# justinruggles/flake

Hardware: AMD Instinct MI355X
Metric: Msamples/s encoded, 16-bit stereo 44.1k blocksize 4096 LPC-8 (higher is better)
Workload: dtype int64/f64; 1 GPU; configs[1]: stereo 16-bit 44.1 kHz, blocksize 4096, LPC max order 8 (level-5 params, order method MAX, partition orders 0-5, stereo estimate), synthetic resonator PCM resident in HBM; frames_per_gpu=4096, batches=one resident batch, outputs=subframe info + packed Rice residual sections, parallelism=frame-sharded x1

## Files before the change

flake_amd/csrc/k3_common.h:

```cpp
#pragma once

#include "device_util.h"

namespace fhip {
namespace {

constexpr int ENC_WWORDS = 2048;

__device__ __forceinline__ int clamp_porder(int porder, int n, int order)
{
    int lim = ilog2_dev((uint32_t)(n ^ (n - 1)));
    porder = min(porder, lim);
    if (order > 0) porder = min(porder, ilog2_dev((uint32_t)(n / order)));
    return porder;
}

constexpr int HIST = 32;

template <int C, int T>
struct SmpImg {
    static constexpr bool V4 = (C % 4 == 0);
    static constexpr int CS = V4 ? 4 : 1;
    static constexpr int COL0 = (16 % C == 0) ? HIST / C : (36 + C - 1) / C;
    static constexpr int ROWS = V4 ? C / 4 : C;
    static constexpr int S = T + COL0 + (V4 ? 1 : 2);
    static constexpr int SIZE = ROWS * S * CS;
    __host__ __device__ static constexpr int at(int col, int r)
    {
        return V4 ? ((r / 4) * S + col) * 4 + (r % 4) : r * S + col;
    }
    __host__ __device__ static constexpr int off(int c)
    {
        return at((c - (((c % C) + C) % C)) / C + COL0, ((c % C) + C) % C);
    }
};

struct FastLds {
    int32_t *smp;
    unsigned long long *sums;
    int32_t *kpar;
    double *coefd;
    unsigned long long *wtot;
    uint32_t *lvl_bits, *lvl_meth;
    int32_t *coef;
    int32_t *misc;
    uint32_t *trial;
    uint32_t *bits;
};

__host__ __device__ inline int fast_window_words(int n, bool wide = false)
{
    int w = 256;
    if (wide) { while (w < 2 * ENC_WWORDS && w < n) w <<= 1; return w; }
    while (w < ENC_WWORDS && 2 * w < n) w <<= 1;
    return w;
}
__host__ __device__ inline bool fast_wide_window(int mode, int bps) { return mode == 2 && bps > 16; }

__host__ __device__ inline size_t fast_lds_layout(int n, size_t img_doubles, size_t off[11], bool wide = false)
{
    size_t o = 0;
    off[0] = o; o += 8 * 512;
    off[1] = o; o += 8 * 48;
    off[2] = o; o += 8 * 16;
    off[3] = o; o += 4 * img_doubles;
    off[4] = o; o += 4 * 512;
    off[5] = o; o += 4 * 12;
    off[6] = o; o += 4 * 12;
    off[7] = o; o += 4 * 32;
    off[8] = o; o += 4 * 16;
    off[9] = o; o += 4 * 32;
    o = (o + 15) & ~(size_t)15;
    off[10] = o; o += 4 * fast_window_words(n, wide);
    return o;
}

constexpr int clog2(int v) { return v <= 1 ? 0 : 1 + clog2(v >> 1); }
constexpr int clog2_up(int v) { return clog2(v) + ((v & (v - 1)) ? 1 : 0); }

template <int C, int T>
struct FastCtx {
    FastLds l;
    int n, i0, tid, lane, wv;
    int obits, precision, pmin_req, pmax_req;
};

template <int C, int T, int OBMAX = 8>
__device__ __forceinline__ void fir_lpc(const FastCtx<C, T> &e, int32_t (&r)[C], int order, int shift)
{
    using Img = SmpImg<C, T>;
    const FastLds &l = e.l;
    const double inv = __builtin_ldexp(1.0, -shift);
    constexpr int OB = (C % 8 == 0 && OBMAX >= 8) ? 8 : (C % 4 == 0) ? 4 : (C % 3 == 0) ? 3 : (C % 5 == 0) ? 5 : (C % 7 == 0) ? 7 : 1;
    constexpr int TB = (16 % C == 0) ? 16 : C * ((8 + C - 1) / C);
    const int32_t *mine = l.smp + e.tid * Img::CS;
#pragma unroll
    for (int ob = 0; ob < C; ob += OB) {
        __builtin_amdgcn_sched_barrier(0);
        double acc[OB];
#pragma unroll
        for (int o = 0; o < OB; o++) acc[o] = 0.0;
#pragma unroll 1
        for (int tb = 0; tb < order; tb += TB) {
            const int32_t *base = mine - (tb / C) * Img::CS;
#pragma unroll
            for (int sb = 0; sb < TB; sb += 8) {
                constexpr int dummy = 0; (void)dummy;
                if (order > tb + sb) {
                    const int NT_ = (TB - sb < 8) ? TB - sb : 8;
                    double W[OB + 7];
                    constexpr int WTOP = Img::V4 ? 7 : -1;
                    if constexpr (Img::V4) {
                        static_assert(!Img::V4 || OB % 4 == 0, "aligned windows");
#pragma unroll
                        for (int m4 = 0; m4 < OB + 7; m4 += 4) {
                            const int4 v = *reinterpret_cast<const int4 *>(base + Img::off(ob - sb - 8 + m4));
                            W[m4] = (double)v.x;
                            if (m4 + 1 < OB + 7) W[m4 + 1] = (double)v.y;
                            if (m4 + 2 < OB + 7) W[m4 + 2] = (double)v.z;
                            if (m4 + 3 < OB + 7) W[m4 + 3] = (double)v.w;
                        }
                    } else {
#pragma unroll
                        for (int m = 0; m < OB + 7; m++)
                            if (m < OB + NT_ - 1) W[m] = (double)base[Img::off(ob - sb - NT_ + m)];
                    }
#ifdef FHIP_FIR_TRIM64
                    const int left = order - (tb + sb);
#else
                    constexpr int left = 8;
#endif
#pragma unroll
                    for (int jj = 0; jj < 8; jj++) {
                        if (jj < NT_ && jj < left) {
                            const double cd = l.coefd[tb + sb + jj];
#pragma unroll
                            for (int o = 0; o < OB; o++)
                                acc[o] = __builtin_fma(cd, W[o + (WTOP >= 0 ? WTOP : NT_ - 1) - jj], acc[o]);
                        }
                    }
                }
            }
        }
#pragma unroll
        for (int o = 0; o < OB; o++) {
            const double z = __builtin_fma(acc[o], inv, 6755399441055744.0);
            const uint32_t qlo = (uint32_t)__double2loint(z);
            uint32_t x;
            if constexpr (Img::V4) {
                const int4 v = *reinterpret_cast<const int4 *>(mine + Img::off(ob + (o & ~3)));
                x = (uint32_t)((o & 3) == 0 ? v.x : (o & 3) == 1 ? v.y : (o & 3) == 2 ? v.z : v.w);
            } else {
                x = (uint32_t)mine[Img::off(ob + o)];
            }
            r[ob + o] = (int32_t)(x - qlo);
        }
    }
    if (e.i0 < order) {
#pragma unroll
        for (int o = 0; o < C; o++)
            if (e.i0 + o < order) r[o] = mine[Img::off(o)];
    }
}

template <int C, int T>
__device__ __forceinline__ void fir_lpc_o8(const FastCtx<C, T> &e, int32_t (&r)[C], int order, int shift,
                                           const double *__restrict__ cd)
{
    using Img = SmpImg<C, T>;
    const double inv = __builtin_ldexp(1.0, -shift);
    constexpr int OB = (C % 8 == 0) ? 8 : (C % 4 == 0) ? 4 : (C % 3 == 0) ? 3 : (C % 5 == 0) ? 5 : (C % 7 == 0) ? 7 : 1;
    const int32_t *mine = e.l.smp + e.tid * Img::CS;
    double cf[8];
#pragma unroll
    for (int jj = 0; jj < 8; jj++) cf[jj] = cd[jj];
#pragma unroll
    for (int ob = 0; ob < C; ob += OB) {
        __builtin_amdgcn_sched_barrier(0);
        double acc[OB];
#pragma unroll
        for (int o = 0; o < OB; o++) acc[o] = 0.0;
        double W[OB + 7];
        if constexpr (Img::V4) {
#pragma unroll
            for (int m4 = 0; m4 < OB + 7; m4 += 4) {
                const int4 v = *reinterpret_cast<const int4 *>(mine + Img::off(ob - 8 + m4));
                W[m4] = (double)v.x;
                if (m4 + 1 < OB + 7) W[m4 + 1] = (double)v.y;
                if (m4 + 2 < OB + 7) W[m4 + 2] = (double)v.z;
                if (m4 + 3 < OB + 7) W[m4 + 3] = (double)v.w;
            }
        } else {
#pragma unroll
            for (int m = 0; m < OB + 7; m++) W[m] = (double)mine[Img::off(ob - 8 + m)];
        }
#pragma unroll
        for (int jj = 0; jj < 8; jj++)
#pragma unroll
            for (int o = 0; o < OB; o++)
                acc[o] = __builtin_fma(cf[jj], W[o + 7 - jj], acc[o]);
#pragma unroll
        for (int o = 0; o < OB; o++) {
            const double z = __builtin_fma(acc[o], inv, 6755399441055744.0);
            const uint32_t qlo = (uint32_t)__double2loint(z);
            uint32_t x;
            if constexpr (Img::V4) {
                const int4 v = *reinterpret_cast<const int4 *>(mine + Img::off(ob + (o & ~3)));
                x = (uint32_t)((o & 3) == 0 ? v.x : (o & 3) == 1 ? v.y : (o & 3) == 2 ? v.z : v.w);
            } else {
                x = (uint32_t)mine[Img::off(ob + o)];
            }
            r[ob + o] = (int32_t)(x - qlo);
        }
    }
    if (e.i0 < order) {
#pragma unroll
        for (int o = 0; o < C; o++)
            if (e.i0 + o < order) r[o] = mine[Img::off(o)];
    }
}

template <int C, int T, int TAPS>
__device__ __forceinline__ void fir_lpc_o16(const FastCtx<C, T> &e, int32_t (&r)[C], int order, int shift,
                                            const double *__restrict__ cd)
{
    using Img = SmpImg<C, T>;
// ... 102 lines not shown
```

flake_amd/csrc/k3_encode.hip:

```cpp
#include "device_util.h"
#include "k3_common.h"

#ifdef FHIP_STAMPS
FHIP_DEFINE_STAMP_READER(fhip_debug_read_stamps_k3)
extern "C" int fhip_debug_read_stamps_k1(long long *out);
extern "C" __attribute__((visibility("default"))) int fhip_debug_read_stamps(long long *out)
{
    long long k1[64];
    int rc = fhip_debug_read_stamps_k3(out);
    if (rc == 0) rc = fhip_debug_read_stamps_k1(k1);
    for (int i = 40; i < 64 && rc == 0; i++) out[i] = k1[i];
    return rc;
}
#endif

namespace fhip {
namespace {

struct EncLds {
    int32_t *smp;
    unsigned long long *sums;
    int32_t *kpar;
    uint32_t *lvl_bits;
    uint32_t *lvl_meth;
// ... 1210 lines not shown
            if (ST >= 1) v += row_shl_u64<1>(v);
            if (ST >= 2) v += row_shl_u64<2>(v);
            if (ST >= 3) v += row_shl_u64<4>(v);
            if (ST >= 4) v += row_shl_u64<8>(v);
            if (ST >= 5) v += __shfl_down(v, 16, WAVE);
            if (writer) s5[k * 32 + (tid >> ST)] = v;
        }
    }
    __syncthreads();
    const int pmax_all = clamp_porder(e.pmax_req, n, min_order);
    if (pmax_all <= 3) {
        const int row = lane >> 4, ll = lane & 15;
        for (int slot0 = e.wv * 4; min_order + slot0 <= max_order; slot0 += NW * 4) {
            const int k = min_order + slot0 + row;
            const bool valid = k <= max_order;
            const int kc = min(k, max_order);
            unsigned long long *heap = heaps + (kc - min_order) * 64;
            unsigned long long v = 0;
            if (valid && ll < 8) v = s5[kc * 32 + 4 * ll] + s5[kc * 32 + 4 * ll + 1] + s5[kc * 32 + 4 * ll + 2] + s5[kc * 32 + 4 * ll + 3];
            const bool leaf = valid && ll < 8;
            if (leaf) heap[7 + ll] = v;
            v += row_shl_u64<1>(v); if (leaf && (ll & 1) == 0) heap[3 + (ll >> 1)] = v;
            v += row_shl_u64<2>(v); if (leaf && (ll & 3) == 0) heap[1 + (ll >> 2)] = v;
            v += row_shl_u64<4>(v); if (leaf && ll == 0) heap[0] = v;
            __builtin_amdgcn_fence(__ATOMIC_RELEASE, "wavefront");
            __builtin_amdgcn_wave_barrier();
            const int L = ilog2_dev((uint32_t)n);
            const int lq = (kc == 0) ? 31 : (kc == 1) ? L : (kc == 2) ? L - 1 : (kc == 3) ? ((n >= (3 << (L - 1))) ? L - 1 : L - 2) : L - 2;
            const int lim = min(ilog2_dev((uint32_t)(n ^ (n - 1))), lq);
            const int pmin = min(e.pmin_req, lim), pmax = min(e.pmax_req, lim);
            const int p = ilog2_dev((uint32_t)(ll + 1));
            uint32_t b = 0;
            int kk = 0;
            const unsigned long long hs = heap[min(ll, 14)];
            const unsigned long long total = heap[0];
            if (valid && ll < 15 && p >= pmin && p <= pmax) {
                const int jn = ll + 1 - (1 << p);
                const int cnt = (n >> p) - (jn == 0 ? kc : 0);
                if (total < 0xFFE00000ull && cnt > 0) kk = rice_k_u32_nb((uint32_t)hs, (uint32_t)cnt, &b);
                else kk = (hs >> 32) ? rice_k_fast(hs, cnt, &b) : rice_k_fast_u32((uint32_t)hs, cnt, &b);
            }
            if (valid) l.kpar[64 + kc * 64 + ll] = kk;
            uint32_t sc = b;
            sc += dpp_u32<0x111>(sc); sc += dpp_u32<0x112>(sc); sc += dpp_u32<0x114>(sc); sc += dpp_u32<0x118>(sc);
            uint32_t big = kk > 14 ? 1u : 0u;
            uint32_t bs = big;
            bs += dpp_u32<0x111>(bs); bs += dpp_u32<0x112>(bs); bs += dpp_u32<0x114>(bs); bs += dpp_u32<0x118>(bs);
            const int base = lane & ~15;
            uint32_t best = 0, method = 0;
            int bp = pmin;
#pragma unroll
            for (int q = 0; q < 4; q++) {
                const uint32_t hi = (uint32_t)__shfl((int)sc, base + (2 << q) - 2, WAVE);
                const uint32_t lo = q ? (uint32_t)__shfl((int)sc, base + (1 << q) - 2, WAVE) : 0u;
                const uint32_t bh = (uint32_t)__shfl((int)bs, base + (2 << q) - 2, WAVE);
                const uint32_t bl = q ? (uint32_t)__shfl((int)bs, base + (1 << q) - 2, WAVE) : 0u;
                const uint32_t bb = hi - lo + 4u * (1u << q);
                if (q >= pmin && q <= pmax && (q == pmin || bb <= best)) { best = bb; bp = q; method = (bh != bl) ? 1u : 0u; }
            }
            if (valid && ll == 0) {
                l.kpar[4 * kc + 0] = (int32_t)((uint32_t)(kc * e.obits + 2) + best + method + 4u);
                l.kpar[4 * kc + 1] = bp;
                l.kpar[4 * kc + 2] = (int32_t)method;
            }
        }
    } else
    for (int k = min_order + e.wv; k <= max_order; k += NW) {
        const int pmin = clamp_porder(e.pmin_req, n, k);
        const int pmax = clamp_porder(e.pmax_req, n, k);
        unsigned long long *heap = heaps + (k - min_order) * 64;
        unsigned long long v = (lane < 32) ? s5[k * 32 + lane] : 0ull;
#define HEAP_STORE(S_) do { if (lane < 32 && (lane & ((1 << (S_)) - 1)) == 0) heap[(1 << (5 - (S_))) - 1 + (lane >> (S_))] = v; } while (0)
        HEAP_STORE(0);
        v += row_shl_u64<1>(v); HEAP_STORE(1);
        v += row_shl_u64<2>(v); HEAP_STORE(2);
        v += row_shl_u64<4>(v); HEAP_STORE(3);
        v += row_shl_u64<8>(v); HEAP_STORE(4);
        v += __shfl_down(v, 16, WAVE); HEAP_STORE(5);
#undef HEAP_STORE
        __builtin_amdgcn_fence(__ATOMIC_RELEASE, "wavefront");
        __builtin_amdgcn_wave_barrier();
        const int p = ilog2_dev((uint32_t)(lane + 1));
        uint32_t b = 0;
        int kk = 0;
        const unsigned long long hs = heap[min(lane, 62)];
        const unsigned long long total = heap[0];
        if (lane < 63 && p >= pmin && p <= pmax) {
            const int jn = lane + 1 - (1 << p);
            const int cnt = (n >> p) - (jn == 0 ? k : 0);
            if (total < 0xFFE00000ull && cnt > 0) kk = rice_k_u32_nb((uint32_t)hs, (uint32_t)cnt, &b);
            else kk = (hs >> 32) ? rice_k_fast(hs, cnt, &b) : rice_k_fast_u32((uint32_t)hs, cnt, &b);
        }
        if (lane < 64) l.kpar[64 + k * 64 + lane] = kk;
        const uint32_t sc = wave_incl_scan_u32_dpp(b);
        const unsigned long long bigm = __ballot(kk > 14);
        uint32_t best = 0, method = 0;
        int bp = pmin;
#pragma unroll
        for (int q = 0; q < 6; q++) {
            const uint32_t hi = (uint32_t)__builtin_amdgcn_readlane((int)sc, (2 << q) - 2);
            const uint32_t lo = q ? (uint32_t)__builtin_amdgcn_readlane((int)sc, (1 << q) - 2) : 0u;
            const unsigned long long lvl = ((1ull << ((2 << q) - 1)) - 1) & ~((1ull << ((1 << q) - 1)) - 1);
            const uint32_t bb = hi - lo + 4u * (1u << q);
            if (q >= pmin && q <= pmax && (q == pmin || bb <= best)) { best = bb; bp = q; method = (bigm & lvl) ? 1u : 0u; }
        }
        if (lane == 0) {
            l.kpar[4 * k + 0] = (int32_t)((uint32_t)(k * e.obits + 2) + best + method + 4u);
            l.kpar[4 * k + 1] = bp;
            l.kpar[4 * k + 2] = (int32_t)method;
        }
    }
    __syncthreads();
    int best = min_order;
    uint32_t best_bits = (uint32_t)__builtin_amdgcn_readfirstlane(l.kpar[4 * min_order]);
    for (int k = min_order + 1; k <= max_order; k++) {
        const uint32_t bits = (uint32_t)__builtin_amdgcn_readfirstlane(l.kpar[4 * k]);
        if (bits < best_bits) { best_bits = bits; best = k; }
    }
    const int best_p = __builtin_amdgcn_readfirstlane(l.kpar[4 * best + 1]);
    const int best_m = __builtin_amdgcn_readfirstlane(l.kpar[4 * best + 2]);
    __syncthreads();
    if (tid < 64) l.kpar[tid] = l.kpar[64 + best * 64 + tid];
    __syncthreads();
    *bits_out = best_bits;
    *porder_out = best_p;
    *method_out = best_m;
    return best;
}

__device__ __forceinline__ void put_bits32(uint32_t *win, int nw, long long pos, int len, uint32_t val)
{
    const long long wi = pos >> 5;
    const int off = (int)(pos & 31);
    const int room = 32 - off;
    if (len <= room) {
        if (wi >= 0 && wi < nw) atomicOr(&win[wi], val << (room - len));
    } else {
        const int spill = len - room;
        if (wi >= 0 && wi < nw) atomicOr(&win[wi], val >> spill);
        if (wi + 1 >= 0 && wi + 1 < nw) atomicOr(&win[wi + 1], val << (32 - spill));
    }
}

template <int C, int T, int MODE>
__device__ __forceinline__
void encode_pow2_body(const fhip_params &P, const int n, const int32_t *__restrict__ smp_all,
                      const int32_t *__restrict__ coefs_all, const int32_t *__restrict__ shift_all,
                      const int32_t *__restrict__ opt_all, const int32_t *__restrict__ fin_all,
                      fhip_subframe_info *__restrict__ info, const fhip_subframe_info *__restrict__ prep,
                      int32_t *__restrict__ res_out, uint8_t *__restrict__ bits_out, const long long slot_bytes,
                      const int narrow_ok, const int s)
{
    extern __shared__ __attribute__((aligned(16))) unsigned char lds_raw[];
    size_t off[12];
    fast_lds_layout(n, SmpImg<C, T>::SIZE, off, fast_wide_window(MODE, P.bits_per_sample));
    FastCtx<C, T> e;
    e.l.sums = reinterpret_cast<unsigned long long *>(lds_raw + off[0]);
    e.l.coefd = reinterpret_cast<double *>(lds_raw + off[1]);
    e.l.wtot = reinterpret_cast<unsigned long long *>(lds_raw + off[2]);
    e.l.smp = reinterpret_cast<int32_t *>(lds_raw + off[3]);
    e.l.kpar = reinterpret_cast<int32_t *>(lds_raw + off[4]);
    e.l.lvl_bits = reinterpret_cast<uint32_t *>(lds_raw + off[5]);
    e.l.lvl_meth = reinterpret_cast<uint32_t *>(lds_raw + off[6]);
    e.l.coef = reinterpret_cast<int32_t *>(lds_raw + off[7]);
    e.l.misc = reinterpret_cast<int32_t *>(lds_raw + off[8]);
    e.l.trial = reinterpret_cast<uint32_t *>(lds_raw + off[9]);
    e.l.bits = reinterpret_cast<uint32_t *>(lds_raw + off[10]);
    const FastLds &l = e.l;

    asm volatile("s_setreg_imm32_b32 hwreg(HW_REG_MODE, 2, 2), 2" ::: "memory");

    const int tid = threadIdx.x;
    e.n = n; e.tid = tid; e.lane = tid & 63;
    e.wv = __builtin_amdgcn_readfirstlane(tid >> 6);
    e.i0 = tid * C;
    e.precision = P.lpc_precision;
    e.pmin_req = P.min_partition_order;
    e.pmax_req = P.max_partition_order;

    constexpr bool MULTI = MODE != 0 && MODE != 3;
    constexpr bool HAS_LPC = MODE != 1;
    constexpr bool pre_row = !MULTI;

    int32_t xn[C];
    int32_t first_n, obits_n, fcoef_n = 0, fshift_n = 0, forder_n = 0, fcabs_n = 0, magbits_n = -1;
    {
        const int32_t *srcp = smp_all + (size_t)s * n;
        const int nflag = (C % 8 == 0 && narrow_ok) ? (prep[s].reserved & 0xFF) : 0;
        const bool narrow = nflag != 0;
        magbits_n = nflag - 1;
        if (C % 8 == 0 && narrow) {
            const int4 *src4 = reinterpret_cast<const int4 *>(reinterpret_cast<const int16_t *>(srcp) + e.i0);
#pragma unroll
            for (int q = 0; q < C / 8; q++) {
                const int4 t4 = src4[q];
                xn[8 * q] = (int32_t)(int16_t)t4.x;     xn[8 * q + 1] = t4.x >> 16;
                xn[8 * q + 2] = (int32_t)(int16_t)t4.y; xn[8 * q + 3] = t4.y >> 16;
                xn[8 * q + 4] = (int32_t)(int16_t)t4.z; xn[8 * q + 5] = t4.z >> 16;
                xn[8 * q + 6] = (int32_t)(int16_t)t4.w; xn[8 * q + 7] = t4.w >> 16;
            }
            first_n = (int32_t)*reinterpret_cast<const int16_t *>(srcp);
        } else if (C % 4 == 0) {
            const int4 *src4 = reinterpret_cast<const int4 *>(srcp + e.i0);
#pragma unroll
            for (int q = 0; q < C / 4; q++) {
                const int4 t4 = src4[q];
                xn[4 * q] = t4.x; xn[4 * q + 1] = t4.y; xn[4 * q + 2] = t4.z; xn[4 * q + 3] = t4.w;
            }
        } else {
#pragma unroll
            for (int q = 0; q < C; q++) xn[q] = srcp[tid + T * q];
        }
        if (!narrow) first_n = srcp[0];
        obits_n = prep[s].obits;
        if (pre_row) {
            const int32_t *f = fin_all + (size_t)s * FIN_STRIDE;
            fcoef_n = f[tid & 31];
            fshift_n = f[32];
            forder_n = f[33];
            fcabs_n = f[34];
        }
    }
  {
    fhip_subframe_info *out = &info[s];
    e.obits = obits_n;
    const int fshift = fshift_n, forder = forder_n;

    STAMP(0);
    int differs = 0;
    {
        const int32_t first = first_n;
        int32_t mx = first, mn = first;
#pragma unroll
        for (int o = 0; o < C; o++) {
            const int32_t v = xn[o];
            if (C % 4 != 0)
                l.smp[SmpImg<C, T>::at((tid + T * o) / C + SmpImg<C, T>::COL0, (tid + T * o) % C)] = v;
            mx = max(mx, v);
            mn = min(mn, v);
        }
        differs = (mx != mn);
        if constexpr (C % 4 == 0) {
#pragma unroll
            for (int g4 = 0; g4 < C; g4 += 4)
                *reinterpret_cast<int4 *>(l.smp + tid * 4 + SmpImg<C, T>::off(g4)) =
                    make_int4(xn[g4], xn[g4 + 1], xn[g4 + 2], xn[g4 + 3]);
        }
    }
    if (tid < SmpImg<C, T>::COL0 * C) l.smp[SmpImg<C, T>::at(tid / C, tid % C)] = 0;
    const int wwords = fast_window_words(n, fast_wide_window(MODE, P.bits_per_sample));
    if (bits_out) for (int q = tid; q < wwords / 4; q += T) reinterpret_cast<uint4 *>(l.bits)[q] = make_uint4(0, 0, 0, 0);
    if (tid < 16) l.coefd[32 + tid] = 0.0;
    if (pre_row && tid < FHIP_MAX_ORDER) {
        l.coef[tid] = fcoef_n;
        l.coefd[tid] = (double)fcoef_n;
    }
    if constexpr (MODE == 3 && C % 8 == 0) {
        const int32_t other = __shfl_xor(fcoef_n, 1, WAVE);
        if (tid < 16 && (tid & 1) == 0) l.trial[tid >> 1] = (uint32_t)((other & 0xFFFF) | (fcoef_n << 16));
    }
    const int wave_differs = (__ballot(differs) != 0ull) ? 1 : 0;
    if (e.lane == 0) l.misc[e.wv] = wave_differs;
    __syncthreads();
    int any_differs = 0;
#pragma unroll
    for (int w = 0; w < T / WAVE; w++) any_differs |= l.misc[w];
    const bool constant = (__builtin_amdgcn_readfirstlane(any_differs) == 0);
    STAMP(1);

    int32_t r[C];
    uint32_t u[C];
    int type, type_code, order = 0, shift = 0;
    uint32_t est_bits = 0;
    bool has_rice = false;
    const int32_t *crow_base = coefs_all + (size_t)s * FHIP_MAX_ORDER * FHIP_MAX_ORDER;
    const int32_t *srow = shift_all + (size_t)s * FHIP_MAX_ORDER;

    enum { T_CONST, T_VERB, T_FIXED, T_LPC } tree;
    if (constant) tree = T_CONST;
    else if (!MULTI) tree = T_LPC;
    else if (MODE == 1) tree = T_FIXED;
    else if (n < 5 || P.prediction_type == 0) tree = T_VERB;
    else if (P.prediction_type == 1 || n <= P.max_prediction_order) tree = T_FIXED;
    else tree = T_LPC;

    const int omethod = MULTI ? P.order_method : 0;
    const int min_order = P.min_prediction_order;
    const int max_order = (tree == T_FIXED) ? min(P.max_prediction_order, 4) : P.max_prediction_order;

    int it = 0, best = 0;
    uint32_t best_bits = 0, last_bits = 0;
    bool have_best = false;
    int lg_step = 16, lg_last = 0, lg_pos = 3;
    bool final_pass = false;
    int porder = 0, method = 0;
    uint32_t umax_run = 0;

    if (tree == T_FIXED) { it = min_order; best = min_order; }
    bool five_wide = false;
    if constexpr (MODE == 1) {
        if (tree == T_FIXED && max_order > min_order && max_order <= 4 && min_order >= 0 &&
            P.max_partition_order <= 5) {
            five_wide = true;
        }
    }
    if (HAS_LPC && tree == T_LPC) {
        if (omethod <= 1) { best = forder - 1; final_pass = true; }
        else if (omethod <= 4) { it = (1 << ((omethod - 1) & 7)) - 1; best = max_order - 1; }
        else if (omethod == 5) { it = 0; best = 0; }
        else {
            best = min_order - 1 + (max_order - min_order) / 3;
            if (tid < FHIP_MAX_ORDER) l.trial[tid] = 0xFFFFFFFFu;
            __syncthreads();
            lg_step = 32;
        }
    }

    if (tree == T_CONST || tree == T_VERB) {
        type = type_code = (tree == T_CONST) ? FHIP_SUB_CONSTANT : FHIP_SUB_VERBATIM;
        est_bits = (uint32_t)(tree == T_CONST ? e.obits : e.obits * n);
    } else {
        if constexpr (MODE == 1) {
            if (five_wide) {
                STAMP(2);
                best = fixed_search5<C, T>(e, min_order, max_order, &est_bits, &porder, &method);
                STAMP(3);
                fir_fixed<C, T>(e, r, best);
                fold_residuals<C, T>(e, r, u, best);
                umax_run = 0;
#pragma unroll
                for (int o = 0; o < C; o++) umax_run = max(umax_run, u[o]);
                STAMP(8);
            }
        }
        if (!five_wide) for (;;) {
            int cand = -1;
            if (!final_pass) {
                if (tree == T_FIXED) {
                    if (it <= max_order) cand = it;
                } else if (omethod <= 4) {
                    if (it >= 0) {
                        const int levels = 1 << ((omethod - 1) & 7);
                        cand = min_order + (((max_order - min_order + 1) * (it + 1)) / levels) - 2;
                        if (cand < 0) cand = 0;
                    }
                } else if (omethod == 5) {
                    if (it < max_order) cand = it;
                } else {
                    for (;;) {
                        if (lg_pos == 3) {
                            lg_step >>= 1;
                            if (lg_step == 0) break;
                            lg_last = best;
                            lg_pos = 0;
                        }
                        const int i = lg_last + (lg_pos - 1) * lg_step;
                        lg_pos++;
                        if (i < min_order - 1 || i >= max_order || l.trial[i] < 0xFFFFFFFFu) continue;
                        cand = i;
                        break;
                    }
                }
                if (cand < 0) {
                    if (tree == T_FIXED && best == max_order) { est_bits = last_bits; break; }
                    final_pass = true;
                }
            }
            if (final_pass) cand = best;

            uint32_t b = 0;
            if (MULTI && (!HAS_LPC || tree == T_FIXED)) {
                fir_fixed<C, T>(e, r, cand);
                __syncthreads();
                b = rice_search_fast<C, T>(e, r, u, cand, false, &porder, &method, &umax_run);
            } else if constexpr (HAS_LPC) {
                const int ord = cand + 1;
                int cshift;
                if (pre_row) {
                    cshift = fshift;
                } else {
                    __syncthreads();
                    if (tid < FHIP_MAX_ORDER) {
                        const int32_t cv = (tid < ord) ? crow_base[cand * FHIP_MAX_ORDER + tid] : 0;
                        l.coef[tid] = cv;
                        l.coefd[tid] = (double)cv;
                        if constexpr (C % 8 == 0) {
                            const int32_t nb = __shfl_xor(cv, 1, WAVE);
                            if (tid < 16 && (tid & 1) == 0) l.misc[tid >> 1] = (nb & 0xFFFF) | (cv << 16);
                            int32_t sa = cv < 0 ? -cv : cv;
                            sa += __shfl_xor(sa, 1, WAVE); sa += __shfl_xor(sa, 2, WAVE);
                            sa += __shfl_xor(sa, 4, WAVE); sa += __shfl_xor(sa, 8, WAVE);
                            sa += __shfl_xor(sa, 16, WAVE);
                            if (tid == 0) l.misc[8] = sa;
                        }
                    }
                    cshift = srow[cand];
                    __syncthreads();
                }
                STAMP(2);
                bool done = false;
                if constexpr (C % 8 == 0) {
                    if (pre_row && ord <= 8 && magbits_n >= 0 &&
                        ((unsigned long long)(uint32_t)fcabs_n << magbits_n) < (1ull << 31)) {
                        fir_lpc_dot8<C, T>(e, r, ord, cshift, fin_all + (size_t)s * FIN_STRIDE + FIN_PAIRS);
                        done = true;
                    }
                    if constexpr (MODE == 3) {
                        if (!done && ord <= 16 && magbits_n >= 0 &&
                            ((unsigned long long)(uint32_t)fcabs_n << magbits_n) < (1ull << 31)) {
                            fir_lpc_dotn<C, T, 8>(e, r, ord, cshift, reinterpret_cast<const int32_t *>(l.trial));
                            done = true;
                        }
                    }
                    if (!pre_row && ord <= 16 && magbits_n >= 0 &&
                        ((unsigned long long)(uint32_t)l.misc[8] << magbits_n) < (1ull << 31)) {
                        if (ord <= 8) fir_lpc_dotn<C, T, 4>(e, r, ord, cshift, l.misc);
                        else fir_lpc_dotn<C, T, 8>(e, r, ord, cshift, l.misc);
                        done = true;
                    }
                }
                if (done) {
                } else if (pre_row && ord <= 8)
                    fir_lpc_o8<C, T>(e, r, ord, cshift,
                                     reinterpret_cast<const double *>(fin_all + (size_t)s * FIN_STRIDE + FIN_DBL));
                else if constexpr (MODE != 0) {
                    bool wide_done = false;
                    if constexpr (MODE == 3 && C % 8 == 0) {
                        const double *cd = reinterpret_cast<const double *>(fin_all + (size_t)s * FIN_STRIDE + FIN_DBL);
                        if (ord <= 12) { fir_lpc_o16<C, T, 12>(e, r, ord, cshift, cd); wide_done = true; }
                        else if (ord <= 16) { fir_lpc_o16<C, T, 16>(e, r, ord, cshift, cd); wide_done = true; }
                    }
                    if (!wide_done) fir_lpc<C, T, (MODE == 3) ? 4 : 8>(e, r, ord, cshift);
                }
                STAMP(3);
                b = rice_search_fast<C, T, (MODE == 2 || MODE == 3)>(e, r, u, ord, true, &porder, &method, &umax_run);
                STAMP(8);
            }
            if (final_pass) { est_bits = b; break; }

            last_bits = b;
            if (tree == T_FIXED) {
                if (!have_best || b < best_bits) { best_bits = b; best = cand; }
                it++;
            } else if (omethod <= 4) {
                if (!have_best) best_bits = b;
                else if (b < best_bits) { best_bits = b; best = cand; }
                it--;
            } else if (omethod == 5) {
                if (!have_best || b < best_bits) { best_bits = b; best = cand; }
                it++;
            } else {
                if (tid == 0) l.trial[cand] = b;
                __syncthreads();
                if (b < l.trial[best]) best = cand;
            }
            have_best = true;

        }
        if (tree == T_FIXED) {
            order = best;
            type = FHIP_SUB_FIXED;
            type_code = FHIP_SUB_FIXED | order;
        } else {
            order = best + 1;
            shift = pre_row ? fshift : srow[best];
            type = FHIP_SUB_LPC;
            type_code = FHIP_SUB_LPC | (order - 1);
        }
        has_rice = true;
    }

    if (!has_rice) { porder = 0; method = 0; }

    STAMP(9);
    if (res_out) {
        const int32_t *mine_s = l.smp + tid * SmpImg<C, T>::CS;
#pragma unroll
        for (int o = 0; o < C; o++) {
            const int32_t back = (int32_t)((u[o] >> 1) ^ (0u - (u[o] & 1u)));
            r[o] = (!has_rice || e.i0 + o < order) ? mine_s[SmpImg<C, T>::off(o)] : back;
        }
        if (C % 4 == 0) {
            int4 *dst4 = reinterpret_cast<int4 *>(res_out + (size_t)s * n + e.i0);
#pragma unroll
            for (int q = 0; q < C / 4; q++)
                dst4[q] = make_int4(r[4 * q], r[4 * q + 1], r[4 * q + 2], r[4 * q + 3]);
        } else {
            int32_t *dst = res_out + (size_t)s * n + e.i0;
#pragma unroll
            for (int o = 0; o < C; o++) dst[o] = r[o];
        }
    }

    long long total_bits = 0;
    if (has_rice) {
        constexpr int LT = clog2(T);
        const int pbits = 4 + method;
        const int heap0 = (1 << porder) - 1;
        const int tpp = LT - porder;
        const int part = tid >> tpp;
        const int k = l.kpar[heap0 + part];
        const int k1 = k + 1;
        const bool part_head = (part > 0) && ((tid & ((1 << tpp) - 1)) == 0);
        const int nwarm = min(max(order - e.i0, 0), C);
        uint32_t umax = umax_run;
        if (__any((umax >> 31) != 0u)) {
            umax = 0;
#pragma unroll
            for (int o = 0; o < C; o++) {
                u[o] = emit_fold32((int32_t)((u[o] >> 1) ^ (0u - (u[o] & 1u)))) & ((e.i0 + o < order) ? 0u : ~0u);
                umax = max(umax, u[o]);
            }
        }
        const uint32_t longest = umax >> k;
        const bool short_codes = !__any(longest + (uint32_t)k1 > 32u);
        const bool tiny_codes = (C % 2 == 0) && !__any(longest + (uint32_t)k1 > 16u);
        unsigned long long mine = (part_head ? pbits : 0) + (unsigned long long)((C - nwarm) * k1);
        if (short_codes) {
            uint32_t m32 = 0;
#pragma unroll
            for (int o = 0; o < C; o++) m32 += u[o] >> k;
            mine += m32;
        } else {
#pragma unroll
            for (int o = 0; o < C; o++) mine += (unsigned long long)(u[o] >> k);
        }
        unsigned long long incl;
        if (__any(mine >> 24)) incl = wave_incl_scan_u64(mine, e.lane);
        else incl = wave_incl_scan_u32_dpp((uint32_t)mine);
        if (e.lane == 63) l.wtot[e.wv] = incl;
        __syncthreads();
        unsigned long long base = 6 + pbits;
        unsigned long long tot = 6 + pbits;
#pragma unroll
        for (int w = 0; w < T / WAVE; w++) {
            const unsigned long long wt = l.wtot[w];
            if (w < e.wv) base += wt;
            tot += wt;
        }
        const unsigned long long my_off = base + incl - mine;
        total_bits = (tot > 0x7FFFFFFFull) ? 0x7FFFFFFFll : (long long)tot;
        STAMP(10);

        if (bits_out) {
            if (tot > (unsigned long long)slot_bytes * 8ull) {
                total_bits = -1;
            } else {
                uint32_t *dst32 = reinterpret_cast<uint32_t *>(bits_out + (size_t)s * slot_bytes);
                const int nwords = (int)((tot + 31) >> 5);
                const long long start = (long long)my_off - (long long)(nwarm * k1);
                for (int wlo = 0; wlo < nwords; wlo += wwords) {
                    const int nw = min(wwords, nwords - wlo);
                    if (wlo > 0) {
                        __syncthreads();
                        for (int q = tid; q < (nw + 3) / 4; q += T) reinterpret_cast<uint4 *>(l.bits)[q] = make_uint4(0, 0, 0, 0);
                        __syncthreads();
                    }
                    const long long rel = start - (long long)wlo * 32;
                    uint32_t hi = 0;
                    int nacc = (int)(rel & 31);
                    int w = (int)(rel >> 5);
                    auto field = [&](int len, uint32_t val) {
                        const uint32_t a = val << ((32 - len) & 31);
                        const uint32_t head = a >> nacc;
                        const uint32_t tail = __builtin_amdgcn_alignbit(a, 0u, (uint32_t)nacc);
                        const int t = nacc + len;
                        const uint32_t word = hi | head;
                        const bool full = t >= 32;
                        if (full && (unsigned)w < (unsigned)nw) atomicOr(&l.bits[w], word);
                        hi = full ? tail : word;
                        w += full ? 1 : 0;
                        nacc = t & 31;
                    };
                    const bool touches = (nwords <= wwords) ||
                                         (rel + (long long)(nwarm * k1) + (long long)mine > 0 && rel < (long long)nw * 32);
                    if (touches) {
                    if (part_head) field(pbits, (uint32_t)k);
                    const uint32_t kmask = (1u << k) - 1u, kbit = 1u << k;
                    bool packed = false;
                    if constexpr (C % 2 == 0) { if (tiny_codes) {
                        packed = true;
#pragma unroll
                        for (int o = 0; o < C; o += 2) {
                            const int l1 = (int)(u[o + 1] >> k) + k1;
                            const uint32_t v0 = (u[o] & kmask) | kbit, v1 = (u[o + 1] & kmask) | kbit;
                            field((int)(u[o] >> k) + k1 + l1, (v0 << l1) | v1);
                        }
                    } }
                    if (packed) {
                    } else if (short_codes) {
#pragma unroll
                        for (int o = 0; o < C; o++)
                            field((int)(u[o] >> k) + k1, (u[o] & kmask) | kbit);
                    } else {
#pragma unroll 2
                        for (int o = 0; o < C; o++) {
                            const uint32_t q = u[o] >> k;
                            if (q >= 32u) {
                                const long long adv = (long long)nacc + q;
                                if (hi && (unsigned)w < (unsigned)nw) atomicOr(&l.bits[w], hi);
                                hi = 0;
                                w += (int)(adv >> 5);
                                nacc = (int)(adv & 31);
                            } else {
                                field((int)q, 0u);
                            }
                            field(k1, (u[o] & kmask) | kbit);
                        }
                    }
                    if (nacc > 0 && hi && (unsigned)w < (unsigned)nw) atomicOr(&l.bits[w], hi);
                    }
                    __syncthreads();
                    if (tid == 0 && wlo == 0) {
                        const int hb = 6 + pbits;
                        const uint32_t hdr = ((uint32_t)method << (4 + pbits)) | ((uint32_t)porder << pbits) |
                                             (uint32_t)l.kpar[heap0];
                        l.bits[0] = (l.bits[0] & (0xFFFFFFFFu >> hb)) | (hdr << (32 - hb));
                    }
                    STAMP(11);
                    const int nq = nw >> 2;
                    for (int q = tid; q < nq; q += T) {
                        const uint4 v = reinterpret_cast<const uint4 *>(l.bits)[q];
                        reinterpret_cast<uint4 *>(dst32 + wlo)[q] =
                            make_uint4(__builtin_bswap32(v.x), __builtin_bswap32(v.y),
                                       __builtin_bswap32(v.z), __builtin_bswap32(v.w));
                    }
                    if (tid < (nw & 3)) dst32[wlo + 4 * nq + tid] = __builtin_bswap32(l.bits[4 * nq + tid]);
                }
            }
        }
    }
    STAMP(12);

    if (tid == 0) {
        out->type = type;
        out->type_code = type_code;
        out->order = order;
        out->shift = shift;
        out->rice_method = method;
        out->porder = porder;
        out->est_bits = est_bits;
        out->rice_nbits = (int32_t)total_bits;
        out->reserved = 0;
        out->obits = prep[s].obits;
        out->wasted = prep[s].wasted;
        out->ch_mode = prep[s].ch_mode;
    }
    if (tid < FHIP_MAX_ORDER) {
        out->coefs[tid] = (type == FHIP_SUB_LPC && tid < order) ? l.coef[tid] : 0;
        const int nw = (type == FHIP_SUB_CONSTANT) ? 1 : order;
        out->warmup[tid] = (tid < nw) ? l.smp[SmpImg<C, T>::at(tid / C + SmpImg<C, T>::COL0, tid % C)] : 0;
    }
    {
        const int np = has_rice ? (1 << porder) : 0;
        for (int q = tid; q < FHIP_MAX_PARTS; q += T) out->rparams[q] = (q < np) ? l.kpar[np - 1 + q] : 0;
    }
  }
}

template <int C, int T, int MODE>
__global__ __launch_bounds__(T, (MODE == 2 || C >= 18 || (C >= 14 && T > 256)) ? 4 : 5)
void k_encode_pow2(fhip_params P, int n, int nsub, const int32_t *__restrict__ smp_all,
                   const int32_t *__restrict__ coefs_all, const int32_t *__restrict__ shift_all,
                   const int32_t *__restrict__ opt_all, const int32_t *__restrict__ fin_all,
                   fhip_subframe_info *__restrict__ info, const fhip_subframe_info *__restrict__ prep,
                   int32_t *__restrict__ res_out, uint8_t *__restrict__ bits_out, long long slot_bytes,
                   int narrow_ok, const int32_t *__restrict__ dev_sub)
{
    if (dev_sub && (int)blockIdx.x >= dev_count(dev_sub, 0)) return;
    encode_pow2_body<C, T, MODE>(P, n, smp_all, coefs_all, shift_all, opt_all, fin_all, info, prep, res_out, bits_out,
                                 slot_bytes, narrow_ok, (int)blockIdx.x);
}

template <int MODE>
__global__ __launch_bounds__(256, 5)
void k_encode_bins(fhip_params P, MultiBin mb, const int32_t *__restrict__ smp,
                   const int32_t *__restrict__ coefs_all, const int32_t *__restrict__ shift_all,
                   const int32_t *__restrict__ opt_all, const int32_t *__restrict__ fin_all,
                   fhip_subframe_info *__restrict__ info, const fhip_subframe_info *__restrict__ prep,
                   uint8_t *__restrict__ bits)
{
    constexpr int T = 256;
    const int blk = blockIdx.x;
    const int k = find_bin(mb, blk);
    const int local = blk - mb.wg0[k];
    if (local >= __builtin_amdgcn_readfirstlane(mb.cnt[mb.cnt_ix[k]])) return;
    const int n = mb.n[k];
    const int s = mb.unit0[k] + local;
    const int32_t *smp_k = smp + mb.smp_off[k] - (long long)mb.unit0[k] * n;
    const long long slot = mb.slot[k];
    uint8_t *bits_k = bits + mb.bits_off[k] - (long long)mb.unit0[k] * slot;
    const int nar = mb.narrow[k];
#define BODY_(CC) encode_pow2_body<CC, T, MODE>(P, n, smp_k, coefs_all, shift_all, opt_all, fin_all, info, prep, nullptr, bits_k, slot, nar, s)
    const int c = n / T;
    if (c == 2) BODY_(2); else if (c == 4) BODY_(4); else if (c == 8) BODY_(8); else if (c == 10) BODY_(10);
    else if (c == 12) BODY_(12); else if (c == 14) BODY_(14); else BODY_(16);
#undef BODY_
}

}

size_t encode_lds_bytes(int n)
{
    if (n < 1 || n > FHIP_MAX_BLOCK) return 0;
    size_t off[10];
    return enc_lds_layout(n > FHIP_MAX_RESIDENT_BLOCK ? 0 : n, off);
}

bool fast_geometry(const fhip_params &p, int n, int *C, int *T)
{
    if (n < 192 || n > FHIP_MAX_BLOCK) return false;
    int odd = n, lg = 0;
    while ((odd & 1) == 0) { odd >>= 1; lg++; }
    int c, t;
    if (odd == 1) {
        if (n >= 4096) { c = 16; t = n / 16; }
        else if (n >= 2048) { c = 8; t = 256; }
        else if (n >= 1024) { c = 4; t = 256; }
        else if (n == 512) {
            c = 8; t = 64;
            if ((n >> p.max_partition_order) < 8 && (n >> p.max_partition_order) >= 2) { c = 2; t = 256; }
        }
        else if (n == 256) { c = 4; t = 64; }
        else return false;
    } else if (odd == 9) {
        c = 9; t = 1 << lg;
        if (t >= 512) { c = 18; t >>= 1; }
    } else if (odd == 3) {
        c = 3; t = 1 << lg;
        if (t > 1024) { c = 6; t >>= 1; }
        if (t > 1024) { c = 0; }
        if (lg == 10 || lg == 11) { c = 12; t = 1 << (lg - 2); }
        if (lg == 9) { c = 6; t = 256; }
    } else if ((odd == 5 || odd == 7) && (lg == 9 || lg == 10)) {
        c = 2 * odd; t = 1 << (lg - 1);
    } else {
        return false;
    }
    if (const char *g = getenv("FHIP_K3_GEOM")) {
        int gc = 0, gt = 0;
        if (sscanf(g, "%d,%d", &gc, &gt) == 2 && gc * gt == n) { c = gc; t = gt; }
    }
    if (c == 0 || t < 64 || t > 1024) return false;
    if ((n >> p.max_partition_order) < c && odd == 1) return false;
    *C = c; *T = t;
    return true;
}

bool narrow_rows_ok(const fhip_params &p, int nsub, int n, bool lpc_path, bool wave_typed_k1)
{
    static const bool off = getenv("FHIP_NO_NARROW") != nullptr || getenv("FHIP_K3_GENERIC") != nullptr;
    if (off || p.channels != 2 || (n & 3) != 0 || n > 8192) return false;
    int fc = 0, ft = 0;
    if (!fast_geometry(p, n, &fc, &ft) || (fc % 8) != 0) return false;
    if (lpc_path && !wave_typed_k1 && !autocorr_is_wave_typed(nsub, n, p.max_prediction_order)) return false;
    return true;
}

int encode_group(const fhip_params &p, int n, bool order_known)
{
    static const bool generic = getenv("FHIP_K3_GENERIC") != nullptr;
    int fc = 0, ft = 0;
    if (generic || !fast_geometry(p, n, &fc, &ft)) return -1;
    const bool single_row = (p.prediction_type == 2) && (n > p.max_prediction_order) && (p.order_method <= 1 || order_known);
    if (!single_row) return -1;
    if (ft == 256 && (fc == 2 || fc == 4 || fc == 8 || fc == 10 || fc == 12 || fc == 14 || fc == 16)) return 256;
    return -1;
}

hipError_t launch_encode_bins(hipStream_t st, const fhip_params &p, const MultiBin &mb, const int32_t *smp,
                              const int32_t *coefs, const int32_t *shift, const int32_t *opt_order, const int32_t *fin,
                              fhip_subframe_info *info, const fhip_subframe_info *prep, uint8_t *bits)
{
    if (mb.nbins < 1) return hipSuccess;
    const int grid = mb.wg0[mb.nbins];
    if (grid == 0) return hipSuccess;
    if (!prep || prep == info) return hipErrorInvalidValue;
    const int mode = (p.max_prediction_order > 8) ? 3 : 0;
    size_t lds = 0;
    for (int k = 0; k < mb.nbins; k++) {
        int fc = 0, ft = 0;
        if (encode_group(p, mb.n[k], true) != 256 || !fast_geometry(p, mb.n[k], &fc, &ft)) return hipErrorInvalidValue;
        size_t off[12], img = 0;
#define SZ_(CC) if (fc == CC) img = (size_t)SmpImg<CC, 256>::SIZE
        SZ_(2); SZ_(4); SZ_(8); SZ_(10); SZ_(12); SZ_(14); SZ_(16);
#undef SZ_
        const size_t l = fast_lds_layout(mb.n[k], img, off, fast_wide_window(mode, p.bits_per_sample));
        lds = l > lds ? l : lds;
    }
#define LAUNCH_EB(MM)                                                                        \
    do {                                                                                     \
        hipError_t er = hipFuncSetAttribute(reinterpret_cast<const void *>(&k_encode_bins<MM>), \
                                            hipFuncAttributeMaxDynamicSharedMemorySize, (int)lds); \
        if (er != hipSuccess) return er;                                                     \
        hipLaunchKernelGGL((k_encode_bins<MM>), dim3(grid), dim3(256), lds, st, p, mb, smp, coefs, shift, opt_order, \
                           fin, info, prep, bits);                                           \
        return hipGetLastError();                                                            \
    } while (0)
    if (mode == 3) LAUNCH_EB(3);
    LAUNCH_EB(0);
#undef LAUNCH_EB
}

hipError_t launch_encode(hipStream_t st, const fhip_params &p, const int32_t *smp,
                         int nsub, int n, const int32_t *coefs, const int32_t *shift,
                         const int32_t *opt_order, const int32_t *fin,
                         fhip_subframe_info *info,
                         int32_t *residual, uint8_t *bits, int64_t slot_bytes,
                         int raw_order, int raw_lpc, bool narrow_ok, const fhip_subframe_info *prep,
                         bool order_known, const int32_t *dev_sub)
{
    if (nsub == 0) return hipSuccess;
    if (!prep || prep == info) return hipErrorInvalidValue;
    int fc = 0, ft = 0;
    static const bool force_generic = getenv("FHIP_K3_GENERIC") != nullptr;
    if (raw_order < 0 && !force_generic && fast_geometry(p, n, &fc, &ft)) {
        size_t off[12];
        size_t lds = 0;
#define LAUNCH_FAST2(CC, TT, MM)                                                             \
    do {                                                                                     \
        lds = fast_lds_layout(n, (size_t)SmpImg<CC, TT>::SIZE, off,                          \
                              fast_wide_window(MM, p.bits_per_sample));                      \
        hipError_t er = hipFuncSetAttribute(                                                 \
            reinterpret_cast<const void *>(&k_encode_pow2<CC, TT, MM>),                      \
            hipFuncAttributeMaxDynamicSharedMemorySize, (int)lds);                           \
        if (er != hipSuccess) return er;                                                     \
        hipLaunchKernelGGL((k_encode_pow2<CC, TT, MM>), dim3(nsub), dim3(TT), lds, st, p, n, \
                           nsub, smp, coefs, shift, opt_order, fin, info, prep, residual,    \
                           bits, (long long)slot_bytes, narrow_ok ? 1 : 0, dev_sub);         \
    } while (0)
        const bool single_row = (p.prediction_type == 2) && (n > p.max_prediction_order) &&
                                (p.order_method <= 1 || order_known);
        const bool fixed_only = (p.prediction_type == 1) && n >= 5;
        const bool wide_rows = p.max_prediction_order > 8;
#define LAUNCH_FAST(CC, TT)                                                                  \
    do {                                                                                     \
        if (single_row && wide_rows) LAUNCH_FAST2(CC, TT, 3);                                \
        else if (single_row) LAUNCH_FAST2(CC, TT, 0);                                        \
        else if (fixed_only) LAUNCH_FAST2(CC, TT, 1);                                        \
        else LAUNCH_FAST2(CC, TT, 2);                                                        \
    } while (0)
        const int key = fc * 10000 + ft;
        switch (key) {
        case 160256: LAUNCH_FAST(16, 256); break;
        case 160512: LAUNCH_FAST(16, 512); break;
        case 161024: LAUNCH_FAST(16, 1024); break;
        case 80256: LAUNCH_FAST(8, 256); break;
        case 40256: LAUNCH_FAST(4, 256); break;
        case 80064: LAUNCH_FAST(8, 64); break;
        case 40064: LAUNCH_FAST(4, 64); break;
        case 20256: LAUNCH_FAST(2, 256); break;
        case 90064: LAUNCH_FAST(9, 64); break;
        case 100256: LAUNCH_FAST(10, 256); break;
        case 100512: LAUNCH_FAST(10, 512); break;
        case 140256: LAUNCH_FAST(14, 256); break;
        case 140512: LAUNCH_FAST(14, 512); break;
        case 180256: LAUNCH_FAST(18, 256); break;
        case 180512: LAUNCH_FAST(18, 512); break;
        case 90128: LAUNCH_FAST(9, 128); break;
        case 90256: LAUNCH_FAST(9, 256); break;
        case 30064: LAUNCH_FAST(3, 64); break;
        case 30128: LAUNCH_FAST(3, 128); break;
        case 30256: LAUNCH_FAST(3, 256); break;
        case 30512: LAUNCH_FAST(3, 512); break;
        case 31024: LAUNCH_FAST(3, 1024); break;
        case 61024: LAUNCH_FAST(6, 1024); break;
        case 60256: LAUNCH_FAST(6, 256); break;
        case 120256: LAUNCH_FAST(12, 256); break;
        case 120512: LAUNCH_FAST(12, 512); break;
        default: return hipErrorInvalidValue;
        }
#undef LAUNCH_FAST
#undef LAUNCH_FAST2
        return hipGetLastError();
    }
    const size_t lds = encode_lds_bytes(n);
    if (lds == 0) return hipErrorInvalidValue;
    if (n > FHIP_MAX_RESIDENT_BLOCK) {
        hipLaunchKernelGGL(k_encode_big, dim3(nsub), dim3(NT), lds, st, p, n, smp, coefs, shift,
                           opt_order, info, prep, residual, bits, (long long)slot_bytes, raw_order,
                           raw_lpc, dev_sub);
        return hipGetLastError();
    }
    const int chunk = (n + NT - 1) / NT;
#define LAUNCH_ENC(CC)                                                                       \
    do {                                                                                     \
        hipError_t er = hipFuncSetAttribute(reinterpret_cast<const void *>(&k_encode<CC>),   \
                                            hipFuncAttributeMaxDynamicSharedMemorySize,      \
                                            (int)lds);                                       \
        if (er != hipSuccess) return er;                                                     \
        hipLaunchKernelGGL(k_encode<CC>, dim3(nsub), dim3(NT), lds, st, p, n, smp, coefs,    \
                           shift, opt_order, info, prep, residual, bits,                     \
                           (long long)slot_bytes,                                            \
                           raw_order, raw_lpc, dev_sub);                                     \
    } while (0)
    if (chunk <= 16) LAUNCH_ENC(16);
    else if (chunk <= 32) LAUNCH_ENC(32);
    else LAUNCH_ENC(64);
#undef LAUNCH_ENC
    return hipGetLastError();
}

}
```

Before: 224,500 Msamples/s.

## Overlay bit window on sample image and shrink heap LDS for single-row mode

For the single-row LPC mode, the LDS bit-output window now shares storage with the sample image, and the partition-sum heaps are sized from max_partition_order instead of a fixed 512 nodes. Warmup samples are saved into the trial array first, and the window is zeroed later, just before residual packing. Launch bounds for C=16,T=256 mode 0 go up to 7 waves per SIMD to use the smaller LDS footprint for more resident blocks. The risks are extra syncs, register pressure from the tighter launch bound, and correctness hazards if the sample image is still read after the overlay is zeroed.

After: 233,800 Msamples/s (median of 6 runs). +4.2%, better.

```diff
diff --git a/flake_amd/csrc/k3_common.h b/flake_amd/csrc/k3_common.h
--- a/flake_amd/csrc/k3_common.h
+++ b/flake_amd/csrc/k3_common.h
@@ -57,21 +57,36 @@
 }
 __host__ __device__ inline bool fast_wide_window(int mode, int bps) { return mode == 2 && bps > 16; }
 
-__host__ __device__ inline size_t fast_lds_layout(int n, size_t img_doubles, size_t off[11], bool wide = false)
-{
+__host__ __device__ inline int fast_heap_nodes(int mode, int max_porder)
+{
+    if (mode != 0) return 512;
+    const int p = max_porder < 0 ? 0 : max_porder > 8 ? 8 : max_porder;
+    return 2 << p;
+}
+__host__ __device__ inline size_t fast_lds_layout(int n, size_t img_doubles, size_t off[11], bool wide = false,
+                                                  int heap_nodes = 512, bool overlay = false)
+{
+    const size_t img_bytes = 4 * img_doubles, win_bytes = 4 * (size_t)fast_window_words(n, wide);
     size_t o = 0;
-    off[0] = o; o += 8 * 512;
+    if (!overlay) { off[0] = o; o += 8 * (size_t)heap_nodes; }
     off[1] = o; o += 8 * 48;
     off[2] = o; o += 8 * 16;
-    off[3] = o; o += 4 * img_doubles;
-    off[4] = o; o += 4 * 512;
+    off[3] = o; o += overlay ? ((img_bytes > win_bytes ? img_bytes : win_bytes) + 15) & ~(size_t)15
+                             : img_bytes;
+    if (!overlay) { off[4] = o; o += 4 * (size_t)heap_nodes; }
     off[5] = o; o += 4 * 12;
     off[6] = o; o += 4 * 12;
     off[7] = o; o += 4 * 32;
     off[8] = o; o += 4 * 16;
     off[9] = o; o += 4 * 32;
     o = (o + 15) & ~(size_t)15;
-    off[10] = o; o += 4 * fast_window_words(n, wide);
+    if (overlay) {
+        off[10] = off[3];
+        off[0] = o; o += 8 * (size_t)heap_nodes;
+        off[4] = o; o += 4 * (size_t)heap_nodes;
+        return o;
+    }
+    off[10] = o; o += win_bytes;
     return o;
 }
 
diff --git a/flake_amd/csrc/k3_encode.hip b/flake_amd/csrc/k3_encode.hip
--- a/flake_amd/csrc/k3_encode.hip
+++ b/flake_amd/csrc/k3_encode.hip
@@ -1386,8 +1386,10 @@
                       const int narrow_ok, const int s)
 {
     extern __shared__ __attribute__((aligned(16))) unsigned char lds_raw[];
+    constexpr bool OVERLAY = MODE == 0;
     size_t off[12];
-    fast_lds_layout(n, SmpImg<C, T>::SIZE, off, fast_wide_window(MODE, P.bits_per_sample));
+    fast_lds_layout(C * T, SmpImg<C, T>::SIZE, off, fast_wide_window(MODE, P.bits_per_sample),
+                    fast_heap_nodes(MODE, P.max_partition_order), OVERLAY);
     FastCtx<C, T> e;
     e.l.sums = reinterpret_cast<unsigned long long *>(lds_raw + off[0]);
     e.l.coefd = reinterpret_cast<double *>(lds_raw + off[1]);
@@ -1483,7 +1485,7 @@
     }
     if (tid < SmpImg<C, T>::COL0 * C) l.smp[SmpImg<C, T>::at(tid / C, tid % C)] = 0;
     const int wwords = fast_window_words(n, fast_wide_window(MODE, P.bits_per_sample));
-    if (bits_out) for (int q = tid; q < wwords / 4; q += T) reinterpret_cast<uint4 *>(l.bits)[q] = make_uint4(0, 0, 0, 0);
+    if (!OVERLAY && bits_out) for (int q = tid; q < wwords / 4; q += T) reinterpret_cast<uint4 *>(l.bits)[q] = make_uint4(0, 0, 0, 0);
     if (tid < 16) l.coefd[32 + tid] = 0.0;
     if (pre_row && tid < FHIP_MAX_ORDER) {
         l.coef[tid] = fcoef_n;
@@ -1500,6 +1502,7 @@
 #pragma unroll
     for (int w = 0; w < T / WAVE; w++) any_differs |= l.misc[w];
     const bool constant = (__builtin_amdgcn_readfirstlane(any_differs) == 0);
+    if (OVERLAY && tid < FHIP_MAX_ORDER) l.trial[tid] = (uint32_t)l.smp[SmpImg<C, T>::at(tid / C + SmpImg<C, T>::COL0, tid % C)];
     STAMP(1);
 
     int32_t r[C];
@@ -1737,6 +1740,10 @@
         const int k1 = k + 1;
         const bool part_head = (part > 0) && ((tid & ((1 << tpp) - 1)) == 0);
         const int nwarm = min(max(order - e.i0, 0), C);
+        if (OVERLAY && bits_out) {
+            if (res_out) __syncthreads();
+            for (int q = tid; q < wwords / 4; q += T) reinterpret_cast<uint4 *>(l.bits)[q] = make_uint4(0, 0, 0, 0);
+        }
         uint32_t umax = umax_run;
         if (__any((umax >> 31) != 0u)) {
             umax = 0;
@@ -1789,6 +1796,10 @@
                         __syncthreads();
                         for (int q = tid; q < (nw + 3) / 4; q += T) reinterpret_cast<uint4 *>(l.bits)[q] = make_uint4(0, 0, 0, 0);
                         __syncthreads();
+                    }
+                    if constexpr (MODE == 0) {
+#pragma unroll
+                        for (int o = 0; o < C; o++) asm volatile("" : "+v"(u[o]));
                     }
                     const long long rel = start - (long long)wlo * 32;
                     uint32_t hi = 0;
@@ -1883,7 +1894,8 @@
     if (tid < FHIP_MAX_ORDER) {
         out->coefs[tid] = (type == FHIP_SUB_LPC && tid < order) ? l.coef[tid] : 0;
         const int nw = (type == FHIP_SUB_CONSTANT) ? 1 : order;
-        out->warmup[tid] = (tid < nw) ? l.smp[SmpImg<C, T>::at(tid / C + SmpImg<C, T>::COL0, tid % C)] : 0;
+        out->warmup[tid] = (tid >= nw) ? 0 : OVERLAY ? (int32_t)l.trial[tid]
+                                                     : l.smp[SmpImg<C, T>::at(tid / C + SmpImg<C, T>::COL0, tid % C)];
     }
     {
         const int np = has_rice ? (1 << porder) : 0;
@@ -1893,7 +1905,7 @@
 }
 
 template <int C, int T, int MODE>
-__global__ __launch_bounds__(T, (MODE == 2 || C >= 18 || (C >= 14 && T > 256)) ? 4 : 5)
+__global__ __launch_bounds__(T, (MODE == 0 && C == 16 && T == 256) ? 7 : (MODE == 2 || C >= 18 || (C >= 14 && T > 256)) ? 4 : 5)
 void k_encode_pow2(fhip_params P, int n, int nsub, const int32_t *__restrict__ smp_all,
                    const int32_t *__restrict__ coefs_all, const int32_t *__restrict__ shift_all,
                    const int32_t *__restrict__ opt_all, const int32_t *__restrict__ fin_all,
@@ -2019,7 +2031,8 @@
 #define SZ_(CC) if (fc == CC) img = (size_t)SmpImg<CC, 256>::SIZE
         SZ_(2); SZ_(4); SZ_(8); SZ_(10); SZ_(12); SZ_(14); SZ_(16);
 #undef SZ_
-        const size_t l = fast_lds_layout(mb.n[k], img, off, fast_wide_window(mode, p.bits_per_sample));
+        const size_t l = fast_lds_layout(mb.n[k], img, off, fast_wide_window(mode, p.bits_per_sample),
+                                         fast_heap_nodes(mode, p.max_partition_order), mode == 0);
         lds = l > lds ? l : lds;
     }
 #define LAUNCH_EB(MM)                                                                        \
@@ -2054,7 +2067,8 @@
 #define LAUNCH_FAST2(CC, TT, MM)                                                             \
     do {                                                                                     \
         lds = fast_lds_layout(n, (size_t)SmpImg<CC, TT>::SIZE, off,                          \
-                              fast_wide_window(MM, p.bits_per_sample));                      \
+                              fast_wide_window(MM, p.bits_per_sample),                       \
+                              fast_heap_nodes(MM, p.max_partition_order), MM == 0);          \
         hipError_t er = hipFuncSetAttribute(                                                 \
             reinterpret_cast<const void *>(&k_encode_pow2<CC, TT, MM>),                      \
             hipFuncAttributeMaxDynamicSharedMemorySize, (int)lds);                           \
```
